# CDCgov/NowcastAutoGP

Hardware: AMD Instinct MI355X
Metric: particle-logml/s (fit+forecast hot path: covariance assembly + Cholesky + logml + predictive per (particle, scenario) item), n=2048 64-particle SMC (higher is better)
Workload: dtype f64

## Files before the change

### nowcastautogp_amd/csrc/ngp_col_kernels.h

```cpp
#pragma once
#include <algorithm>

#include "ngp_mfma.h"

namespace ngp {

struct NoProbe {
    __device__ __forceinline__ void mark(int) {}
    template <class T>
    __device__ __forceinline__ void mark_after(int, T) {}
    __device__ __forceinline__ void drain() {}
    __device__ __forceinline__ void emit_diag(int, int, int) {}
    __device__ __forceinline__ void emit_col(int, int, int, int, int, int, bool) {}
    __device__ __forceinline__ void begin(int, int, int) {}
    __device__ __forceinline__ void sweep(int) {}
};

__device__ __forceinline__ void sqrt_and_rcp(double a, double &d, double &r) {
    double y = __builtin_amdgcn_rsq(a);
    const double h = 0.5 * a;
    y = y * fma(-h * y, y, 1.5);
    y = y * fma(-h * y, y, 1.5);
    d = a * y;
    d = fma(fma(-d, d, a), 0.5 * y, d);
    r = fma(fma(-d, y, 1.0), y, y);
}

__device__ __forceinline__ int tri(int r, int c) { return ((r * (r + 1)) >> 1) + c; }
constexpr int TRI = NB * (NB + 1) / 2;

template <class Probe = NoProbe>
__global__ __launch_bounds__(256, 4) void chol_diag_kernel(JobGeom g, ChunkPtrs p, int j, int k0) {
    __shared__ double Mt[TRI];
    __shared__ double Lt[TRI];
    __shared__ double pan[NB][4];
    __shared__ double dblk[16];
    __shared__ double dinvd[4];
    __shared__ double rdg[NB];
    __shared__ double logs[NB];
    __shared__ double Ts[TB][TB + 1];
    __shared__ int bad;
    const int item = blockIdx.x;
    const int tid = threadIdx.x, lane = tid & 63;
    const int wave = __builtin_amdgcn_readfirstlane(tid >> 6);
    const long ld = g.ld;
    double *Lit = p.L + (long)item * g.item_stride;
    double *Lj = Lit + (long)j * NB * ld;
    const int kmax = j * NB;
    const int r16 = lane & 15, q = lane >> 4;
    const int wr = wave >> 1, wc = wave & 1;
    Probe probe;
    probe.mark_after(0, lane);

    if (tid == 0) bad = 0;

    if (!(wr == 0 && wc == 1)) {
        double acc4[2][2][4];
#pragma unroll
        for (int a = 0; a < 2; ++a)
#pragma unroll
            for (int b = 0; b < 2; ++b)
#pragma unroll
                for (int r = 0; r < 4; ++r) acc4[a][b][r] = 0.0;
        const double *pa = Lj + (long)(32 * wr + r16) * ld + 2 * q;
        const double *pb = Lj + (long)(32 * wc + r16) * ld + 2 * q;
        double kt[2][2][4];
#pragma unroll
        for (int mt = 0; mt < 2; ++mt)
#pragma unroll
            for (int nt = 0; nt < 2; ++nt)
#pragma unroll
                for (int s = 0; s < 4; ++s)
                    kt[mt][nt][s] = Lj[(long)(32 * wr + 16 * mt + q + 4 * s) * ld + kmax +
                                       32 * wc + 16 * nt + r16];
        for (int kc = k0; kc < kmax; kc += 16) {
            double a[2][4], b[2][4];
#pragma unroll
            for (int u = 0; u < 2; ++u) {
                const f64x2 alo = *reinterpret_cast<const f64x2 *>(pa + (long)u * 16 * ld + kc);
                const f64x2 ahi = *reinterpret_cast<const f64x2 *>(pa + (long)u * 16 * ld + kc + 8);
                const f64x2 blo = *reinterpret_cast<const f64x2 *>(pb + (long)u * 16 * ld + kc);
                const f64x2 bhi = *reinterpret_cast<const f64x2 *>(pb + (long)u * 16 * ld + kc + 8);
                a[u][0] = alo.x; a[u][1] = alo.y; a[u][2] = ahi.x; a[u][3] = ahi.y;
                b[u][0] = blo.x; b[u][1] = blo.y; b[u][2] = bhi.x; b[u][3] = bhi.y;
            }
#pragma unroll
            for (int s = 0; s < 4; ++s)
#pragma unroll
                for (int nt = 0; nt < 2; ++nt) {
                    const Rot4 br = rot4(b[nt][s]);
#pragma unroll
                    for (int mt = 0; mt < 2; ++mt) mfma16_as_4(acc4[mt][nt], a[mt][s], br);
                }
        }
        f64x4 acc[2][2];
#pragma unroll
        for (int a = 0; a < 2; ++a)
#pragma unroll
            for (int b = 0; b < 2; ++b) acc[a][b] = to_d16(acc4[a][b]);
#pragma unroll
        for (int mt = 0; mt < 2; ++mt)
#pragma unroll
            for (int nt = 0; nt < 2; ++nt)
#pragma unroll
                for (int s = 0; s < 4; ++s) {
                    const int M = 32 * wr + 16 * mt + q + 4 * s, N = 32 * wc + 16 * nt + r16;
                    if (M >= N) Mt[tri(M, N)] = kt[mt][nt][s] - acc[mt][nt][s];
                }
    }
    __syncthreads();
    probe.mark_after(1, lane);

    const int bi = tid >> 4, bj = tid & 15;
    {
        double a[4][4];
#pragma unroll
        for (int r = 0; r < 4; ++r)
#pragma unroll
            for (int c = 0; c < 4; ++c) {
                const int R = 4 * bi + r, C = 4 * bj + c;
                a[r][c] = (R >= C) ? Mt[tri(R, C)] : 0.0;
            }
        for (int kb = 0; kb < NB / 4; ++kb) {
            if (bi == kb && bj == kb) {
                double dks[4];
#pragma unroll
                for (int kc = 0; kc < 4; ++kc) {
                    const double akk = a[kc][kc];
                    double dk, inv;
                    sqrt_and_rcp(akk, dk, inv);
                    if (!(akk > 0.0) && bad == 0) bad = 4 * kb + kc + 1;
                    dks[kc] = dk;
                    dinvd[kc] = inv;
                    rdg[4 * kb + kc] = inv;
#pragma unroll
                    for (int r = 0; r < 4; ++r)
                        if (r > kc) a[r][kc] *= inv;
#pragma unroll
                    for (int c = 0; c < 4; ++c)
                        if (c > kc) {
#pragma unroll
                            for (int r = 0; r < 4; ++r)
                                if (r >= c) a[r][c] -= a[r][kc] * a[c][kc];
                        }
                }
#pragma unroll
                for (int r = 0; r < 4; ++r)
#pragma unroll
                    for (int c = 0; c < 4; ++c) {
                        if (r == c) a[r][c] = dks[r];
                        if (c > r) a[r][c] = 0.0;
                        dblk[4 * r + c] = a[r][c];
                    }
            }
            __syncthreads();
            if (bj == kb && bi > kb) {
#pragma unroll
                for (int c = 0; c < 4; ++c) {
                    const double inv = dinvd[c];
#pragma unroll
                    for (int r = 0; r < 4; ++r) {
                        double v = a[r][c];
#pragma unroll
                        for (int pp = 0; pp < 4; ++pp)
                            if (pp < c) v -= a[r][pp] * dblk[4 * c + pp];
                        a[r][c] = v * inv;
                    }
                }
#pragma unroll
                for (int r = 0; r < 4; ++r)
#pragma unroll
                    for (int c = 0; c < 4; ++c) pan[4 * bi + r][c] = a[r][c];
            }
            __syncthreads();
            if (bj > kb && bi >= bj) {
                double li[4][4], lj[4][4];
#pragma unroll
                for (int r = 0; r < 4; ++r)
#pragma unroll
                    for (int pp = 0; pp < 4; ++pp) {
                        li[r][pp] = pan[4 * bi + r][pp];
                        lj[r][pp] = pan[4 * bj + r][pp];
                    }
#pragma unroll
                for (int pp = 0; pp < 4; ++pp)
#pragma unroll
                    for (int r = 0; r < 4; ++r)
#pragma unroll
                        for (int c = 0; c < 4; ++c) a[r][c] -= li[r][pp] * lj[c][pp];
            }
        }
#pragma unroll
        for (int r = 0; r < 4; ++r) {
            const int R = 4 * bi + r;
            f64x2 lo, hi;
            lo.x = (R >= 4 * bj) ? a[r][0] : 0.0;
            lo.y = (R >= 4 * bj + 1) ? a[r][1] : 0.0;
            hi.x = (R >= 4 * bj + 2) ? a[r][2] : 0.0;
            hi.y = (R >= 4 * bj + 3) ? a[r][3] : 0.0;
            double *dst = Lj + (long)R * ld + kmax + 4 * bj;
            *reinterpret_cast<f64x2 *>(dst) = lo;
            *reinterpret_cast<f64x2 *>(dst + 2) = hi;
#pragma unroll
            for (int c = 0; c < 4; ++c)
                if (R >= 4 * bj + c) Lt[tri(R, 4 * bj + c)] = a[r][c];
        }
    }
    __syncthreads();
    probe.mark_after(2, lane);
    if (tid < NB) logs[tid] = log(Lt[tri(tid, tid)]);

    if (tid < NB) {
        const int b = tid >> 4, c = tid & 15;
        double x[TB];
#pragma unroll
        for (int i = 0; i < TB; ++i) {
            double sum = (i == c) ? 1.0 : 0.0;
            int off = tri(TB * b + i, TB * b);
            if (i > 0) asm volatile("" : "+v"(off) : "v"(x[i - 1]));
            const double *lrow = &Lt[off];
#pragma unroll
            for (int pp = 0; pp < i; ++pp) sum -= lrow[pp] * x[pp];
            x[i] = sum * rdg[TB * b + i];
        }
#pragma unroll
        for (int i = 0; i < TB; ++i)
            if (i >= c) Mt[tri(TB * b + i, TB * b + c)] = x[i];
    }
    __syncthreads();
    probe.mark_after(3, lane);
    {
        const int ra = tid >> 4, cb = tid & 15;
        for (int dist = 1; dist < NB / TB; ++dist)
            for (int ct = dist; ct < NB / TB; ++ct) {
                const int jt = ct - dist;
                double t = 0.0;
                for (int kt = jt; kt < ct; ++kt)
#pragma unroll
                    for (int pp = 0; pp < TB; ++pp) {
                        const double mv = Mt[tri(TB * kt + pp, TB * jt + cb)];
                        t += Lt[tri(TB * ct + ra, TB * kt + pp)] * ((kt > jt || pp >= cb) ? mv : 0.0);
                    }
                Ts[ra][cb] = t;
                __syncthreads();
                double mv = 0.0;
#pragma unroll
                for (int pp = 0; pp < TB; ++pp) {
                    const double md = Mt[tri(TB * ct + ra, TB * ct + pp)];
                    mv -= ((pp <= ra) ? md : 0.0) * Ts[pp][cb];
                }
                Mt[tri(TB * ct + ra, TB * jt + cb)] = mv;
                __syncthreads();
            }
    }
    probe.mark_after(4, lane);
    {
        double *dv = p.dinv + (long)item * (NB * NB);
        for (int e = tid; e < NB * NB; e += 256) {
            const int strip = e >> 6, l = e & 63;
            const int cb4 = strip >> 2, jt = strip & 3;
            const int R = 4 * cb4 + (l & 3), C = 16 * jt + 4 * ((l >> 2) & 3) + (l >> 4);
            dv[e] = (R >= C) ? Mt[tri(R, C)] : 0.0;
        }
    }
    if (tid == 0) {
        double s = 0.0;
        for (int k = 0; k < NB; ++k) s += logs[k];
        p.logdet[item] += s;
        if (bad && p.info[item] == 0) p.info[item] = kmax + bad;
    }
    probe.mark_after(5, lane);
    probe.emit_diag(j, tid, item);
}

template <int NF>
struct Frag8 {
    f64x2 v[NF];
};
template <int NF>
__device__ __forceinline__ void load_frag8(Frag8<NF> &f, const double *p, long ld) {
#pragma unroll
    for (int u = 0; u < NF; ++u) f.v[u] = *reinterpret_cast<const f64x2 *>(p + (long)u * 16 * ld);
}
template <int NA>
__device__ __forceinline__ void mfma_frag8(double (&acc)[NA][4][4], const Frag8<NA> &a,
                                           const Frag8<4> &b) {
#pragma unroll
    for (int it = 0; it < 4; ++it) {
        const Rot4 br = rot4(b.v[it].x);
#pragma unroll
        for (int jt = 0; jt < NA; ++jt) mfma16_as_4(acc[jt][it], a.v[jt].x, br);
    }
#pragma unroll
    for (int it = 0; it < 4; ++it) {
        const Rot4 br = rot4(b.v[it].y);
#pragma unroll
        for (int jt = 0; jt < NA; ++jt) mfma16_as_4(acc[jt][it], a.v[jt].y, br);
    }
}

template <int NA>
__device__ __forceinline__ void gemm_rows(double (&acc)[NA][4][4], const double *pa,
                                          const double *pb, long ld, int k0, int k1) {
    if (k1 <= k0) return;
    Frag8<NA> a0, a1;
    Frag8<4> b0, b1;
    load_frag8(a0, pa + k0, ld);
    load_frag8(b0, pb + k0, ld);
    for (int kc = k0; kc < k1; kc += 16) {
        load_frag8(a1, pa + kc + 8, ld);
        load_frag8(b1, pb + kc + 8, ld);
        mfma_frag8(acc, a0, b0);
        if (kc + 16 < k1) {
            load_frag8(a0, pa + kc + 16, ld);
            load_frag8(b0, pb + kc + 16, ld);
        }
        mfma_frag8(acc, a1, b1);
    }
}

constexpr int EPI_PITCH = 66;
constexpr int EPI_M_BYTES = NB * NB * 8;
constexpr int EPI_WAVE_BYTES = 16 * EPI_PITCH * 8;
constexpr int EPI_LDS_BYTES = EPI_M_BYTES + 4 * EPI_WAVE_BYTES;

__device__ __forceinline__ void stage_mstrips(double *lds_m, const double *mstrips, int tid) {
#pragma unroll
    for (int i = 0; i < 8; ++i) {
        const int idx = tid + 256 * i;
        reinterpret_cast<f64x2 *>(lds_m)[idx] = reinterpret_cast<const f64x2 *>(mstrips)[idx];
    }
}

template <bool SHADOW = false, bool SYNTH = false, class Probe = NoProbe, bool KROWS = false>
__device__ __forceinline__ void solve_and_store_lds(const double (*acc4)[4][4], double *Lr,
                                                    const double *lds_m, long ld, int kmax,
                                                    int lane, double *buf, Probe &probe,
                                                    float *Lr32 = nullptr,
                                                    float *tmax_out = nullptr, int synth = 0,
                                                    const double *ksl = nullptr, int nit = 4) {
    double amax = 0.0;
    const int n16 = lane & 15, isub = lane >> 4;
    const int jj0 = 4 * (n16 >> 2) + isub;
    const double *ksl0 = ksl ? ksl + 15 - jj0 : nullptr;
    f64x2 kvr[8];
    double kvp[4][4];
    const int hrow = lane >> 5, c2 = 2 * (lane & 31);
    bool from_rows = KROWS && ksl0 == nullptr;
    if constexpr (SYNTH) from_rows = from_rows && synth == 0;
    auto k_elems = [&](int it, double (&kv)[4][4]) {
        if (ksl0) {
#pragma unroll
            for (int jt = 0; jt < 4; ++jt)
#pragma unroll
                for (int r = 0; r < 4; ++r)
                    kv[jt][r] = ksl0[((n16 + 4 * r) & 15) + 16 * (it - jt + 3)];
            return;
        }
        if constexpr (SYNTH) {
            if (synth) {
#pragma unroll
                for (int jt = 0; jt < 4; ++jt)
#pragma unroll
                    for (int r = 0; r < 4; ++r) {
                        const int i = 16 * it + ((n16 + 4 * r) & 15);
                        kv[jt][r] = (synth == 2 && i == 16 * jt + jj0) ? 1.0 : 0.0;
                    }
                return;
            }
        }
        if constexpr (!KROWS) {
#pragma unroll
            for (int jt = 0; jt < 4; ++jt)
#pragma unroll
                for (int r = 0; r < 4; ++r) {
                    const int i = 16 * it + ((n16 + 4 * r) & 15);
                    kv[jt][r] = Lr[(long)i * ld + kmax + 16 * jt + jj0];
                }
        }
    };
    auto load_k = [&](int it) {
        if constexpr (KROWS) {
            if (!from_rows) return;
#pragma unroll
            for (int i = 0; i < 8; ++i)
                kvr[i] = *reinterpret_cast<const f64x2 *>(Lr + (long)(16 * it + 2 * i + hrow) * ld + kmax + c2);
        } else {
            k_elems(it, kvp);
        }
    };
    auto take_k = [&](int it, double (&kv)[4][4]) {
        if constexpr (KROWS) {
            if (!from_rows) {
                k_elems(it, kv);
                return;
            }
#pragma unroll
            for (int i = 0; i < 8; ++i)
                *reinterpret_cast<f64x2 *>(buf + (2 * i + hrow) * EPI_PITCH + c2) = kvr[i];
#pragma unroll
            for (int jt = 0; jt < 4; ++jt)
#pragma unroll
                for (int r = 0; r < 4; ++r)
                    kv[jt][r] = buf[((n16 + 4 * r) & 15) * EPI_PITCH + 16 * jt + jj0];
        } else {
#pragma unroll
            for (int jt = 0; jt < 4; ++jt)
#pragma unroll
                for (int r = 0; r < 4; ++r) kv[jt][r] = kvp[jt][r];
        }
    };
    load_k(0);
#pragma unroll
    for (int it = 0; it < 4; ++it) {
        if (it >= nit) break;
        double c4[4][4];
        take_k(it, c4);
#pragma unroll
        for (int jt = 0; jt < 4; ++jt)
#pragma unroll
            for (int r = 0; r < 4; ++r) c4[jt][r] = c4[jt][r] - acc4[jt][it][r];
        probe.mark_after(12 + 3 * it, c4[3][3] + c4[0][0] + c4[1][2] + c4[2][1]);
        if (it + 1 < nit) load_k(it + 1);
        double ms[2][4];
        ms[0][0] = lds_m[lane];
#pragma unroll
        for (int cb4 = 0; cb4 < 16; ++cb4) {
            const int ct = cb4 >> 2;
            if (cb4 + 1 < 16) {
#pragma unroll
                for (int jt = 0; jt <= ((cb4 + 1) >> 2); ++jt)
                    ms[(cb4 + 1) & 1][jt] = lds_m[((cb4 + 1) * 4 + jt) * 64 + lane];
            }
            double R[4] = {0.0, 0.0, 0.0, 0.0};
#pragma unroll
            for (int jt = 0; jt <= ct; ++jt) {
#pragma unroll
                for (int r = 0; r < 4; ++r) R[r] = mfma4(ms[cb4 & 1][jt], c4[jt][r], R[r]);
            }
            double x = R[0];
            x += dpp_f64<ROW_ROR4, 0xF>(R[1], R[1]);
            x += dpp_f64<ROW_ROR8, 0xF>(R[2], R[2]);
            x += dpp_f64<ROW_ROR12, 0xF>(R[3], R[3]);
            buf[n16 * EPI_PITCH + 4 * cb4 + isub] = x;
        }
        probe.mark_after(13 + 3 * it, it);
#pragma unroll
        for (int w = 0; w < 8; ++w) {
            const int idx = w * 64 + lane, row = idx >> 5, cp = idx & 31;
            const f64x2 v = *reinterpret_cast<const f64x2 *>(buf + row * EPI_PITCH + 2 * cp);
            *reinterpret_cast<f64x2 *>(Lr + (long)(16 * it + row) * ld + kmax + 2 * cp) = v;
            if constexpr (SHADOW) {
                typedef float f32x2 __attribute__((ext_vector_type(2)));
                f32x2 vf;
                vf.x = (float)v.x;
                vf.y = (float)v.y;
                *reinterpret_cast<f32x2 *>(Lr32 + (long)(16 * it + row) * ld + kmax + 2 * cp) = vf;
                amax = fmax(amax, fmax(fabs(v.x), fabs(v.y)));
            }
        }
        probe.mark_after(14 + 3 * it, it);
        __builtin_amdgcn_sched_barrier(0);
    }
    if constexpr (SHADOW) {
#pragma unroll
        for (int off = 32; off > 0; off >>= 1) amax = fmax(amax, __shfl_xor(amax, off, 64));
        if (lane == 0) *tmax_out = __double2float_ru(amax);
    }
}

__device__ __forceinline__ void subtract_in_place_perm(double *rows, long ld, int c0,
                                                       const double (*acc4)[4][4], int lane,
                                                       bool fresh = false,
                                                       const double *ksl = nullptr, int nit = 4) {
    const int n16 = lane & 15, isub = lane >> 4;
    const int jj0 = 4 * (n16 >> 2) + isub;
    double *base = rows + c0 + jj0;
    long roff[4];
#pragma unroll
    for (int r = 0; r < 4; ++r) roff[r] = (long)((n16 + 4 * r) & 15) * ld;
    if (ksl) {
        const double *ksl0 = ksl + 15 - jj0;
#pragma unroll
        for (int it = 0; it < 4; ++it)
#pragma unroll
            for (int jt = 0; jt < 4; ++jt)
#pragma unroll
                for (int r = 0; r < 4; ++r)
                    base[(long)(16 * it) * ld + roff[r] + 16 * jt] =
                        ksl0[((n16 + 4 * r) & 15) + 16 * (it - jt + 3)] - acc4[jt][it][r];
        return;
    }
    if (fresh) {
#pragma unroll
        for (int it = 0; it < 4; ++it)
#pragma unroll
            for (int jt = 0; jt < 4; ++jt)
#pragma unroll
                for (int r = 0; r < 4; ++r)
                    base[(long)(16 * it) * ld + roff[r] + 16 * jt] = -acc4[jt][it][r];
        return;
    }
    double v[2][4][4];
#pragma unroll
    for (int jt = 0; jt < 4; ++jt)
#pragma unroll
        for (int r = 0; r < 4; ++r) v[0][jt][r] = base[roff[r] + 16 * jt];
#pragma unroll
    for (int it = 0; it < 4; ++it) {
        if (it >= nit) break;
        if (it + 1 < nit) {
#pragma unroll
            for (int jt = 0; jt < 4; ++jt)
#pragma unroll
                for (int r = 0; r < 4; ++r)
                    v[(it + 1) & 1][jt][r] = base[(long)(16 * (it + 1)) * ld + roff[r] + 16 * jt];
        }
#pragma unroll
        for (int jt = 0; jt < 4; ++jt)
#pragma unroll
            for (int r = 0; r < 4; ++r)
                base[(long)(16 * it) * ld + roff[r] + 16 * jt] = v[it & 1][jt][r] - acc4[jt][it][r];
    }
}

__device__ __forceinline__ void subtract_in_place_rows(double *rows, long ld, int c0,
                                                       const double (*acc4)[4][4], int lane,
                                                       double *tl, bool fresh = false,
                                                       const double *ksl = nullptr, int nit = 4) {
    const int n16 = lane & 15, isub = lane >> 4;
    const int jj0 = 4 * (n16 >> 2) + isub;
    const int hrow = lane >> 5, c2 = 2 * (lane & 31);
    double *base = rows + c0 + c2;
    auto load_rows = [&](int it, f64x2 (&kv)[8]) {
        if (ksl) {
#pragma unroll
            for (int i = 0; i < 8; ++i) {
                const int d = 63 + 16 * it + 2 * i + hrow - c2;
                kv[i].x = ksl[d];
                kv[i].y = ksl[d - 1];
            }
        } else if (fresh) {
#pragma unroll
            for (int i = 0; i < 8; ++i) kv[i].x = kv[i].y = 0.0;
        } else {
#pragma unroll
            for (int i = 0; i < 8; ++i)
                kv[i] = *reinterpret_cast<const f64x2 *>(base + (long)(16 * it + 2 * i + hrow) * ld);
        }
    };
    f64x2 kv[2][8];
    load_rows(0, kv[0]);
#pragma unroll
    for (int it = 0; it < 4; ++it) {
        if (it >= nit) break;
        if (it + 1 < nit) load_rows(it + 1, kv[(it + 1) & 1]);
#pragma unroll
        for (int jt = 0; jt < 4; ++jt)
#pragma unroll
            for (int r = 0; r < 4; ++r)
                tl[((n16 + 4 * r) & 15) * EPI_PITCH + 16 * jt + jj0] = acc4[jt][it][r];
#pragma unroll
        for (int i = 0; i < 8; ++i) {
            const f64x2 a = *reinterpret_cast<const f64x2 *>(tl + (2 * i + hrow) * EPI_PITCH + c2);
            f64x2 o;
            o.x = kv[it & 1][i].x - a.x;
            o.y = kv[it & 1][i].y - a.y;
            *reinterpret_cast<f64x2 *>(base + (long)(16 * it + 2 * i + hrow) * ld) = o;
        }
    }
}

__device__ __forceinline__ void struct_slice(double *ksl, const JobGeom &g, const ChunkPtrs &p,
                                             int item, int row0, int col0, int lane) {
    const double *tab = p.tab + (long)item * g.maxstat * g.R;
    const int d0 = row0 - col0 - 63;
    ksl[lane] = tab[(long)g.toep * (d0 + lane)];
    if (lane < 63) ksl[64 + lane] = tab[(long)g.toep * (d0 + 64 + lane)];
}
constexpr int TOEP_LDS_BYTES = 4 * 128 * 8;

struct ColStep {
    int j;
    int k0;
    int nmain;
    int ntiles;
    int groups;
    int splits;
    int first_touch;
    double c32, jitter;
};
__device__ __forceinline__ long tmax_index(const JobGeom &g, int row_tile, int col) {
    return (long)row_tile * g.nb0 + col;
}

template <bool MIXED, bool IDENT = false, bool TOEP = false>
__global__ __launch_bounds__(256, 2) void chol_col_kernel(JobGeom g, ChunkPtrs p, int Bc,
                                                          ColStep st) {
    __shared__ __attribute__((aligned(16))) char epi[EPI_LDS_BYTES + (TOEP ? TOEP_LDS_BYTES : 0)];
    const int wg = blockIdx.x;
    const int xcd = wg & 7, idx = wg >> 3;
    const int slot = (idx / st.groups) * 8 + xcd;
    const int grp = idx % st.groups;
    if (slot >= Bc) return;
    const int item = p.items ? p.items[slot] : slot;
    const int tid = threadIdx.x, lane = tid & 63;
    const int wave = __builtin_amdgcn_readfirstlane(tid >> 6);
    const int tile = grp * 4 + wave;
    bool valid = tile < st.ntiles;
    int kbeg = st.k0;
    int synth = 0;
    if constexpr (IDENT) {
        if (valid && tile >= st.nmain) {
            const int a = tile - st.nmain;
            if (a < g.nb0) {
                if (a > st.j) valid = false;
                else if (a * NB > kbeg) kbeg = a * NB;
                synth = (a == st.j) ? 2 : 1;
            }
        }
    }

    const int j = st.j;
    const long ld = g.ld;
    double *Lit = p.L + (long)item * g.item_stride;
    const int kmax = j * NB;
    const int r16 = lane & 15, q = lane >> 4;

    double acc4[4][4][4];
#pragma unroll
    for (int a = 0; a < 4; ++a)
#pragma unroll
        for (int b = 0; b < 4; ++b)
#pragma unroll
            for (int r = 0; r < 4; ++r) acc4[a][b][r] = 0.0;

    const int vt = valid ? tile : 0;
    const long rowbase = (vt < st.nmain) ? (long)(j + 1 + vt) * NB
                                         : (long)g.n0 + (long)(vt - st.nmain) * NB;
    double *Lr = Lit + rowbase * ld;
    const double *Lj = Lit + (long)j * NB * ld;
    const double *pa = Lj + (long)r16 * ld + 2 * q;
    const double *pb = Lr + (long)r16 * ld + 2 * q;
    if (valid) gemm_rows<4>(acc4, pa, pb, ld, kbeg, kmax);
    const double *ksl = nullptr;
    if constexpr (TOEP) {
        if (valid && tile < st.nmain && prog_structure(p.progs + item)) {
            double *sl = reinterpret_cast<double *>(epi + EPI_LDS_BYTES) + wave * 128;
            struct_slice(sl, g, p, item, (int)rowbase, kmax, lane);
            ksl = sl;
        }
    }
    stage_mstrips(reinterpret_cast<double *>(epi), p.dinv + (long)item * (NB * NB), tid);
    __syncthreads();
    if (!valid) return;
    NoProbe probe;
    if constexpr (MIXED) {
        const int rt = (tile < st.nmain) ? j + 1 + tile : g.nb0 + (tile - st.nmain);
        solve_and_store_lds<true>(
            acc4, Lr, reinterpret_cast<const double *>(epi), ld, kmax, lane,
            reinterpret_cast<double *>(epi + EPI_M_BYTES + wave * EPI_WAVE_BYTES), probe,
            p.L32 + (long)item * g.item_stride + rowbase * ld,
            p.tmax + (long)item * (g.nb0 + g.naux_pad / NB) * g.nb0 + tmax_index(g, rt, j));
    } else {
        solve_and_store_lds<false, IDENT>(
            acc4, Lr, reinterpret_cast<const double *>(epi), ld, kmax, lane,
            reinterpret_cast<double *>(epi + EPI_M_BYTES + wave * EPI_WAVE_BYTES), probe, nullptr,
            nullptr, synth, ksl);
    }
}

template <bool MIXED, class Probe = NoProbe, bool IDENT = false>
__global__ __launch_bounds__(256, 2) void chol_col_thin_kernel(JobGeom g, ChunkPtrs p, int Bc,
                                                               ColStep st) {
    constexpr int A_BYTES = NB * NB * 8;
    constexpr int TAIL = (4 * EPI_WAVE_BYTES > A_BYTES) ? 4 * EPI_WAVE_BYTES : A_BYTES;
    __shared__ __attribute__((aligned(1024))) char smem[EPI_M_BYTES + TAIL];
    typedef __attribute__((address_space(3))) void *lds_ptr;
    const int wg = blockIdx.x;
    const int xcd = wg & 7, idx = wg >> 3;
    const int slot = (idx / st.groups) * 8 + xcd;
    const int grp = idx % st.groups;
    if (slot >= Bc) return;
    const int item = p.items ? p.items[slot] : slot;
    const int tid = threadIdx.x, lane = tid & 63;
    const int wave = __builtin_amdgcn_readfirstlane(tid >> 6);
    const int tile = grp * 4 + wave;
    bool valid = tile < st.ntiles;
    const int j = st.j;
    const int kmax = j * NB, k0 = kmax - NB;
    bool update = true;
    int synth = 0;
    if constexpr (IDENT) {
        if (valid && tile >= st.nmain) {
            const int a = tile - st.nmain;
            if (a < g.nb0) {
                if (a > j) valid = false;
                else if (a * NB > k0) update = false;
                if (a == j) synth = 2;
            }
        }
    }
    const long ld = g.ld;
    double *Lit = p.L + (long)item * g.item_stride;
    const int r16 = lane & 15, q = lane >> 4;
    Probe probe;
    probe.mark_after(0, lane);

    {
        const __amdgpu_buffer_rsrc_t rl = __builtin_amdgcn_make_buffer_rsrc(
            Lit, 0, (int)(g.item_stride * (long)sizeof(double)), 0x00020000);
        const __amdgpu_buffer_rsrc_t rm = __builtin_amdgcn_make_buffer_rsrc(
            p.dinv + (long)item * (NB * NB), 0, NB * NB * 8, 0x00020000);
        const int rbit = lane >> 5, sl = lane & 31;
#pragma unroll
        for (int i = 0; i < 8; ++i) {
            const int key = (2 * i + rbit) & 7;
            const unsigned voff = (unsigned)((rbit * ld + 2 * (sl ^ key)) * 8);
            const unsigned soff = (unsigned)__builtin_amdgcn_readfirstlane(
                (int)((((long)kmax + 2 * (8 * wave + i)) * ld + k0) * 8));
            lds_ptr dst = (lds_ptr)(smem + EPI_M_BYTES + (8 * wave + i) * 1024);
            __builtin_amdgcn_raw_ptr_buffer_load_lds(rl, dst, 16, voff, soff, 0, 0);
        }
#pragma unroll
        for (int i = 0; i < 8; ++i) {
            lds_ptr dst = (lds_ptr)(smem + (8 * wave + i) * 1024);
            __builtin_amdgcn_raw_ptr_buffer_load_lds(rm, dst, 16, (unsigned)(lane * 16),
                                                     (unsigned)((8 * wave + i) * 1024), 0, 0);
        }
    }

    double acc4[4][4][4];
#pragma unroll
    for (int a = 0; a < 4; ++a)
#pragma unroll
        for (int b = 0; b < 4; ++b)
#pragma unroll
            for (int r = 0; r < 4; ++r) acc4[a][b][r] = 0.0;

    const int vt = valid ? tile : 0;
    const long rowbase = (vt < st.nmain) ? (long)(j + 1 + vt) * NB
                                         : (long)g.n0 + (long)(vt - st.nmain) * NB;
    double *Lr = Lit + rowbase * ld;
    const double *pb = Lr + (long)r16 * ld + k0 + 2 * q;
    const bool mult = valid && update;
    Frag8<4> b[4];
    if (mult) {
#pragma unroll
        for (int sg = 0; sg < 4; ++sg) load_frag8(b[sg], pb + 8 * sg, ld);
    }
    __syncthreads();
    probe.mark_after(1, lane);
    if (mult) {
        const char *Ab = smem + EPI_M_BYTES + r16 * 512;
        const int key = r16 & 7;
#pragma unroll
        for (int sg = 0; sg < 8; ++sg) {
            Frag8<4> a;
#pragma unroll
            for (int u = 0; u < 4; ++u)
                a.v[u] = *reinterpret_cast<const f64x2 *>(Ab + u * (16 * 512) +
                                                          (((4 * sg + q) ^ key) << 4));
            mfma_frag8(acc4, a, b[sg & 3]);
            if (sg + 4 < 8) load_frag8(b[sg & 3], pb + 8 * (sg + 4), ld);
        }
    }
    probe.mark_after(2, acc4[0][0][0] + acc4[3][3][3]);
    __syncthreads();
    probe.mark_after(3, lane);
    probe.mark_after(4, lane);
    if (!valid) return;
    double *buf = reinterpret_cast<double *>(smem + EPI_M_BYTES + wave * EPI_WAVE_BYTES);
    if constexpr (MIXED) {
        const int rt = (tile < st.nmain) ? j + 1 + tile : g.nb0 + (tile - st.nmain);
        solve_and_store_lds<true, false, Probe, true>(
            acc4, Lr, reinterpret_cast<const double *>(smem), ld, kmax, lane, buf, probe,
            p.L32 + (long)item * g.item_stride + rowbase * ld,
            p.tmax + (long)item * (g.nb0 + g.naux_pad / NB) * g.nb0 + tmax_index(g, rt, j));
    } else {
        int nit = (tile >= st.nmain && g.naux - NB * (tile - st.nmain) <= 16) ? 1 : 4;
        if (IDENT && tile < st.nmain && g.n_real - NB * (j + 1 + tile) <= 16) nit = 1;
        solve_and_store_lds<false, IDENT, Probe, true>(acc4, Lr, reinterpret_cast<const double *>(smem), ld,
                                          kmax, lane, buf, probe, nullptr, nullptr, synth, nullptr,
                                          nit);
    }
    probe.mark_after(5, lane);
    probe.drain();
    probe.mark_after(6, lane);
    probe.emit_col(j, lane, wg, wave, item, tile, true);
}

constexpr int LDS_KC = 16;

typedef float f32x4 __attribute__((ext_vector_type(4)));
typedef float f32x16 __attribute__((ext_vector_type(16)));


template <bool MIXED, class Probe = NoProbe, bool IDENT = false, int SPLITK = 0>
__global__ __launch_bounds__(256, 2) void chol_col_glds_kernel(JobGeom g, ChunkPtrs p, int Bc,
                                                               ColStep st) {
    constexpr int ROWB = 128, BLKB = 8 * ROWB + 128, STAGE = 32 * BLKB;
    auto row_off = [](int row) { return (row >> 3) * BLKB + (row & 7) * ROWB; };
    __shared__ __attribute__((aligned(1024))) char smem[2 * STAGE];
    typedef __attribute__((address_space(3))) void *lds_ptr;

    const int wg = blockIdx.x;
    const int xcd = wg & 7, idx = wg >> 3;
    const int per_item = SPLITK == 1 ? st.groups * st.splits : st.groups;
    const int slot = (idx / per_item) * 8 + xcd;
    const int grp = SPLITK == 1 ? (idx % per_item) / st.splits : idx % st.groups;
    const int piece = SPLITK == 1 ? (idx % per_item) % st.splits : 0;
    if (slot >= Bc) return;
    const int item = (MIXED && p.order) ? p.order[slot] : slot;
    const int tid = threadIdx.x, lane = tid & 63;
    const int wave = __builtin_amdgcn_readfirstlane(tid >> 6);
    const int ltile = wave >> 1, col = wave & 1;
    const int tile0 = grp * 2;
    const int tile = tile0 + ltile;
    bool valid = tile < st.ntiles;

    const int j = st.j;
    Probe probe;
    probe.mark(0);
    const long ld = g.ld;
    double *Lit = p.L + (long)item * g.item_stride;
    const int kmax = j * NB;
    bool structured = false;
    if constexpr (!MIXED && !IDENT) {
        if (g.toep && st.first_touch && valid && tile < st.nmain && !(col && tile == 0))
            structured = prog_structure(p.progs + item) != 0;
    }
    int kbeg = st.k0;
    int synth = 0;
    if constexpr (IDENT) {
        const int a = tile - st.nmain;
        if (tile < st.ntiles && a >= 0 && a < g.nb0) synth = (a == j) ? 2 : 1;
    }
    if (IDENT && tile0 >= st.nmain) {
        int kfirst = kmax + 1;
#pragma unroll
        for (int u = 0; u < 2; ++u) {
            const int a = tile0 + u - st.nmain;
            if (tile0 + u >= st.ntiles) continue;
            const int ks = (a >= g.nb0) ? st.k0 : (a > j) ? kmax + 1 : max(st.k0, a * NB);
            kfirst = min(kfirst, ks);
        }
        if (kfirst > kmax) return;
        kbeg = kfirst;
        const int a = tile - st.nmain;
        if (valid && a < g.nb0 && a > j) valid = false;
    }
    int nit = 4;
    if constexpr (!MIXED && SPLITK == 0) {
        if (IDENT && !valid) nit = 0;
        else if (valid && tile >= st.nmain && g.naux - NB * (tile - st.nmain) <= 16) nit = 1;
        else if (IDENT && valid && tile < st.nmain && g.n_real - NB * (j + 1 + tile) <= 16) nit = 1;
    }
    const int r16 = lane & 15, q = lane >> 4;
    auto tile_row0 = [&](int t) -> long {
        if (t >= st.ntiles) t = st.ntiles - 1;
        return (t < st.nmain) ? (long)(j + 1 + t) * NB : (long)g.n0 + (long)(t - st.nmain) * NB;
    };
    const __amdgpu_buffer_rsrc_t rsrc = __builtin_amdgcn_make_buffer_rsrc(
        Lit, 0, (int)(g.item_stride * (long)sizeof(double)), 0x00020000);
    long src_row0;
    if (wave < 2) src_row0 = (long)j * NB + 64 * wave;
    else src_row0 = tile_row0(tile0 + (wave - 2));
    const unsigned soff_base = (unsigned)__builtin_amdgcn_readfirstlane((int)(src_row0 * ld * 8));
    const unsigned row_step8 = (unsigned)(8 * ld * 8);
    const unsigned voff_even = (unsigned)(((lane >> 3) * ld + 2 * ((lane & 7) ^ ((lane >> 4) & 7))) * 8);
    const unsigned voff_odd = (unsigned)(((lane >> 3) * ld + 2 * ((lane & 7) ^ ((4 + (lane >> 4)) & 7))) * 8);
    auto stage = [&](int buf, int k) {
        const unsigned kb = (unsigned)k * 8u;
#pragma unroll
        for (int i = 0; i < 8; ++i) {
            lds_ptr dst = (lds_ptr)(smem + buf * STAGE + (8 * wave + i) * BLKB);
            __builtin_amdgcn_raw_ptr_buffer_load_lds(rsrc, dst, 16, (i & 1) ? voff_odd : voff_even,
                                                     soff_base + i * row_step8 + kb, 0, 0);
        }
    };
    unsigned a_addr[4], b_addr[4][4];
    {
        const int arow = 64 * col + r16;
        const int akey = (r16 >> 1) & 7;
#pragma unroll
        for (int s = 0; s < 4; ++s)
            a_addr[s] = (unsigned)(row_off(arow) + (((2 * s + (q >> 1)) ^ akey) << 4) + (q & 1) * 8);
#pragma unroll
        for (int r = 0; r < 4; ++r) {
            const int rr = (r16 + 4 * r) & 15;
            const int brow = 128 + 64 * ltile + rr;
            const int bkey = (rr >> 1) & 7;
#pragma unroll
            for (int s = 0; s < 4; ++s)
                b_addr[r][s] =
                    (unsigned)(row_off(brow) + (((2 * s + (q >> 1)) ^ bkey) << 4) + (q & 1) * 8);
        }
    }

    double acc4[4][4][4];
#pragma unroll
    for (int a = 0; a < 4; ++a)
#pragma unroll
        for (int b = 0; b < 4; ++b)
#pragma unroll
            for (int r = 0; r < 4; ++r) acc4[a][b][r] = 0.0;

    auto mult64 = [&](const char *buf, auto nit_c) {
        constexpr int NIT = decltype(nit_c)::value;
#pragma unroll
        for (int s = 0; s < 4; ++s) {
            double a[4];
#pragma unroll
            for (int u = 0; u < 4; ++u)
                a[u] = *reinterpret_cast<const double *>(buf + a_addr[s] + u * 2 * BLKB);
#pragma unroll
            for (int it = 0; it < NIT; ++it) {
                Rot4 br;
                br.r0 = *reinterpret_cast<const double *>(buf + b_addr[0][s] + it * 2 * BLKB);
                br.r1 = *reinterpret_cast<const double *>(buf + b_addr[1][s] + it * 2 * BLKB);
                br.r2 = *reinterpret_cast<const double *>(buf + b_addr[2][s] + it * 2 * BLKB);
                br.r3 = *reinterpret_cast<const double *>(buf + b_addr[3][s] + it * 2 * BLKB);
#pragma unroll
                for (int jt = 0; jt < 4; ++jt) mfma16_as_4(acc4[jt][it], a[jt], br);
            }
        }
    };

    if constexpr (SPLITK == 2) {
    } else if constexpr (!MIXED) {
        int nchunks = (kmax - kbeg) / LDS_KC;
        if constexpr (SPLITK == 1) {
            const int per = (nchunks + st.splits - 1) / st.splits;
            const int c0 = min(piece * per, nchunks);
            nchunks = min(c0 + per, nchunks) - c0;
            kbeg += c0 * LDS_KC;
        }
        if (nchunks > 0) {
            stage(0, kbeg);
            __syncthreads();
            if (IDENT && nit == 0) {
                for (int c = 0; c < nchunks; ++c) {
                    if (c + 1 < nchunks) stage((c & 1) ^ 1, kbeg + (c + 1) * LDS_KC);
                    __syncthreads();
                }
            } else if (nit == 1) {
                for (int c = 0; c < nchunks; ++c) {
                    const int cur = c & 1;
                    if (c + 1 < nchunks) stage(cur ^ 1, kbeg + (c + 1) * LDS_KC);
                    mult64(smem + cur * STAGE, std::integral_constant<int, 1>{});
                    __syncthreads();
                }
            } else {
                for (int c = 0; c < nchunks; ++c) {
                    const int cur = c & 1;
                    if (c + 1 < nchunks) stage(cur ^ 1, kbeg + (c + 1) * LDS_KC);
                    mult_chunk_pipelined<2 * BLKB>(acc4, smem + cur * STAGE, a_addr, b_addr);
                    __syncthreads();
                    if (c == 0) probe.mark(1);
                    if (c == nchunks / 2) probe.mark(2);
                }
            }
        }
    } else {
        const int nkt = j;
        const int nbt = g.nb0 + g.naux_pad / NB;
        const float *tm = p.tmax + (long)item * nbt * g.nb0;
        const int t1 = min(tile0 + 1, st.ntiles - 1);
        const int rt0 = (tile0 < st.nmain) ? j + 1 + tile0 : g.nb0 + (tile0 - st.nmain);
        const int rt1 = (t1 < st.nmain) ? j + 1 + t1 : g.nb0 + (t1 - st.nmain);
        const double lim = st.c32 * (p.progs[item].noise + st.jitter);
        unsigned long long m32lo, m32hi;
        {
            bool c[2];
#pragma unroll
            for (int h = 0; h < 2; ++h) {
                const int kt = lane + 64 * h;
                c[h] = false;
                if (kt < nkt) {
                    const float ta = fmaxf(tm[tmax_index(g, j, kt)], tm[tmax_index(g, j + 1, kt)]);
                    const float tb = fmaxf(tm[tmax_index(g, rt0, kt)], tm[tmax_index(g, rt1, kt)]);
                    c[h] = (double)ta * (double)tb <= lim;
                }
            }
            m32lo = __ballot(c[0]);
            m32hi = __ballot(c[1]);
        }
        const unsigned long long inlo = nkt >= 64 ? ~0ull : ((1ull << nkt) - 1ull);
        const unsigned long long inhi = nkt <= 64 ? 0ull : (nkt >= 128 ? ~0ull : ((1ull << (nkt - 64)) - 1ull));
        unsigned long long m64lo = inlo & ~m32lo, m64hi = inhi & ~m32hi;
        const int n32 = __popcll(m32lo) + __popcll(m32hi);
        const int n64 = __popcll(m64lo) + __popcll(m64hi);
        if (tid == 0 && p.mixcnt) {
            const unsigned nv = (unsigned)(2 * min(2, st.ntiles - tile0));
            atomicAdd(p.mixcnt + 2 * item, nv * (unsigned)n32);
            atomicAdd(p.mixcnt + 2 * item + 1, nv * (unsigned)n64);
        }
        auto pop = [](unsigned long long &lo, unsigned long long &hi) -> int {
            if (lo) {
                const int b = __builtin_ctzll(lo);
                lo &= lo - 1;
                return b;
            }
            const int b = __builtin_ctzll(hi);
            hi &= hi - 1;
            return 64 + b;
        };

        if (n32 > 0) {
            const __amdgpu_buffer_rsrc_t rsrc32 = __builtin_amdgcn_make_buffer_rsrc(
                p.L32 + (long)item * g.item_stride, 0, (int)(g.item_stride * (long)sizeof(float)),
                0x00020000);
            const unsigned soff32 = (unsigned)__builtin_amdgcn_readfirstlane((int)(src_row0 * ld * 4));
            const unsigned row_step32 = (unsigned)(8 * ld * 4);
            const unsigned v32_even = (unsigned)((lane >> 3) * ld * 4 + 16 * ((lane & 7) ^ ((lane >> 4) & 7)));
            const unsigned v32_odd = (unsigned)((lane >> 3) * ld * 4 + 16 * ((lane & 7) ^ ((4 + (lane >> 4)) & 7)));
            auto stage32 = [&](int buf, int k) {
                const unsigned kb = (unsigned)k * 4u;
#pragma unroll
                for (int i = 0; i < 8; ++i) {
                    lds_ptr dst = (lds_ptr)(smem + buf * STAGE + (8 * wave + i) * BLKB);
                    __builtin_amdgcn_raw_ptr_buffer_load_lds(rsrc32, dst, 16,
                                                             (i & 1) ? v32_odd : v32_even,
                                                             soff32 + i * row_step32 + kb, 0, 0);
                }
            };
            const int r32 = lane & 31, h = lane >> 5;
            unsigned a32[2][4], b32[2][4];
#pragma unroll
            for (int blk = 0; blk < 2; ++blk) {
                const int arow = 64 * col + 32 * blk + r32;
                const int brow = 128 + 64 * ltile + 32 * blk + r32;
#pragma unroll
                for (int u = 0; u < 4; ++u) {
                    a32[blk][u] = (unsigned)(row_off(arow) + (((2 * u + h) ^ ((arow >> 1) & 7)) << 4));
                    b32[blk][u] = (unsigned)(row_off(brow) + (((2 * u + h) ^ ((brow >> 1) & 7)) << 4));
                }
            }
            f32x16 acc32[2][2];
            double acc64p[2][2][16];
#pragma unroll
            for (int a = 0; a < 2; ++a)
#pragma unroll
                for (int b = 0; b < 2; ++b)
#pragma unroll
                    for (int v = 0; v < 16; ++v) {
                        acc32[a][b][v] = 0.f;
                        acc64p[a][b][v] = 0.0;
                    }
            unsigned long long lo = m32lo, hi = m32hi;
            const int nch = 2 * n32;
            int kt_cur = pop(lo, hi), sub = 1;
            stage32(0, kt_cur * NB);
            __syncthreads();
            for (int c = 0; c < nch; ++c) {
                const int cur = c & 1;
                if (c + 1 < nch) {
                    if (sub == 2) {
                        kt_cur = pop(lo, hi);
                        sub = 0;
                    }
                    stage32(cur ^ 1, kt_cur * NB + 32 * sub);
                    ++sub;
                }
                const char *buf = smem + cur * STAGE;
#pragma unroll
                for (int u = 0; u < 4; ++u) {
                    f32x4 av[2], bv[2];
#pragma unroll
                    for (int blk = 0; blk < 2; ++blk) {
                        av[blk] = *reinterpret_cast<const f32x4 *>(buf + a32[blk][u]);
                        bv[blk] = *reinterpret_cast<const f32x4 *>(buf + b32[blk][u]);
                    }
#pragma unroll
                    for (int e = 0; e < 4; ++e)
#pragma unroll
                        for (int a = 0; a < 2; ++a)
#pragma unroll
                            for (int b = 0; b < 2; ++b)
                                acc32[a][b] = __builtin_amdgcn_mfma_f32_32x32x2f32(
                                    av[a][e], bv[b][e], acc32[a][b], 0, 0, 0);
                }
                if (c & 1) {
#pragma unroll
                    for (int a = 0; a < 2; ++a)
#pragma unroll
                        for (int b = 0; b < 2; ++b)
#pragma unroll
                            for (int v = 0; v < 16; ++v) {
                                acc64p[a][b][v] += (double)acc32[a][b][v];
                                acc32[a][b][v] = 0.f;
                            }
                }
                __syncthreads();
            }
            constexpr int P64 = 65;
            double *t64 = reinterpret_cast<double *>(smem) + wave * (32 * P64);
            static_assert(4 * 32 * P64 * 8 <= 2 * STAGE, "hand-over tiles must fit the stage buffers");
            const int jj0 = 4 * (r16 >> 2) + q;
#pragma unroll
            for (int a = 0; a < 2; ++a) {
#pragma unroll
                for (int b = 0; b < 2; ++b)
#pragma unroll
                    for (int v = 0; v < 16; ++v)
                        t64[((v & 3) + 8 * (v >> 2) + 4 * h) * P64 + 32 * b + r32] = acc64p[a][b][v];
                __syncthreads();
#pragma unroll
                for (int jl = 0; jl < 2; ++jl)
#pragma unroll
                    for (int it = 0; it < 4; ++it)
#pragma unroll
                        for (int r = 0; r < 4; ++r)
                            acc4[2 * a + jl][it][r] =
                                t64[(16 * jl + jj0) * P64 + 16 * it + ((r16 + 4 * r) & 15)];
                __syncthreads();
            }
        }
        if (n64 > 0) {
            unsigned long long lo = m64lo, hi = m64hi;
            const int nch = 4 * n64;
            int kt_cur = pop(lo, hi), sub = 1;
            stage(0, kt_cur * NB);
            __syncthreads();
            for (int c = 0; c < nch; ++c) {
                const int cur = c & 1;
                if (c + 1 < nch) {
                    if (sub == 4) {
                        kt_cur = pop(lo, hi);
                        sub = 0;
                    }
                    stage(cur ^ 1, kt_cur * NB + LDS_KC * sub);
                    ++sub;
                }
                mult_chunk_pipelined<2 * BLKB>(acc4, smem + cur * STAGE, a_addr, b_addr);
                __syncthreads();
            }
        }
    }
    if constexpr (SPLITK == 1) {
        double *mine = p.splitk_part +
                       ((((long)slot * SPLITK_SLOTS + (long)grp * st.splits + piece) * 4 + wave) *
                        (64 * 64)) + lane;
#pragma unroll
        for (int jt = 0; jt < 4; ++jt)
#pragma unroll
            for (int it = 0; it < 4; ++it)
#pragma unroll
                for (int r = 0; r < 4; ++r) mine[((jt * 4 + it) * 4 + r) * 64] = acc4[jt][it][r];
        return;
    }
    if constexpr (SPLITK == 2) {
        const double *part = p.splitk_part +
                             ((((long)slot * SPLITK_SLOTS + (long)grp * st.splits) * 4 + wave) *
                              (64 * 64)) + lane;
#pragma unroll
        for (int jt = 0; jt < 4; ++jt)
#pragma unroll
            for (int it = 0; it < 4; ++it)
#pragma unroll
                for (int r = 0; r < 4; ++r) acc4[jt][it][r] = part[((jt * 4 + it) * 4 + r) * 64];
        for (int q2 = 1; q2 < st.splits; ++q2) {
            const double *pq = part + (long)q2 * 4 * (64 * 64);
            double v[4][4][4];
#pragma unroll
            for (int jt = 0; jt < 4; ++jt)
#pragma unroll
                for (int it = 0; it < 4; ++it)
#pragma unroll
                    for (int r = 0; r < 4; ++r) v[jt][it][r] = pq[((jt * 4 + it) * 4 + r) * 64];
#pragma unroll
            for (int jt = 0; jt < 4; ++jt)
#pragma unroll
                for (int it = 0; it < 4; ++it)
#pragma unroll
                    for (int r = 0; r < 4; ++r) acc4[jt][it][r] += v[jt][it][r];
        }
    }
    static_assert(EPI_LDS_BYTES + TOEP_LDS_BYTES <= 2 * STAGE,
                  "epilogue LDS must fit the stage buffers");
    probe.mark(3);
    const double *ksl = nullptr;
    if (structured) {
        double *sl = reinterpret_cast<double *>(smem + EPI_LDS_BYTES) + wave * 128;
        struct_slice(sl, g, p, item, (int)tile_row0(tile), col ? kmax + NB : kmax, lane);
        ksl = sl;
    }
    stage_mstrips(reinterpret_cast<double *>(smem), p.dinv + (long)item * (NB * NB), tid);
    __syncthreads();
    probe.mark(4);
    if (!valid) return;

    double *Lr = Lit + tile_row0(tile) * ld;
    if (col) {
        subtract_in_place_rows(Lr, ld, (j + 1) * NB, acc4, lane,
                               reinterpret_cast<double *>(smem + EPI_M_BYTES + wave * EPI_WAVE_BYTES),
                               IDENT && synth != 0, ksl, nit);
    } else if constexpr (MIXED) {
        const int rt = (tile < st.nmain) ? j + 1 + tile : g.nb0 + (tile - st.nmain);
        solve_and_store_lds<true>(
            acc4, Lr, reinterpret_cast<const double *>(smem), ld, kmax, lane,
            reinterpret_cast<double *>(smem + EPI_M_BYTES + wave * EPI_WAVE_BYTES), probe,
            p.L32 + (long)item * g.item_stride + tile_row0(tile) * ld,
            p.tmax + (long)item * (g.nb0 + g.naux_pad / NB) * g.nb0 + tmax_index(g, rt, j));
    } else {
        solve_and_store_lds<false, IDENT>(
            acc4, Lr, reinterpret_cast<const double *>(smem), ld, kmax, lane,
            reinterpret_cast<double *>(smem + EPI_M_BYTES + wave * EPI_WAVE_BYTES), probe, nullptr,
            nullptr, synth, ksl, nit);
    }
    probe.mark(5);
    probe.drain();
    probe.mark(6);
    probe.emit_col(j, lane, wg, wave, item, tile, false);
}

template <class Probe>
void launch_chol_diag_t(const JobGeom &g, const ChunkPtrs &p, int Bc, int j, int k0, hipStream_t s) {
    hipLaunchKernelGGL(chol_diag_kernel<Probe>, dim3(Bc), dim3(256), 0, s, g, p, j, k0);
}

template <class Probe>
void launch_chol_col_t(const JobGeom &g, const ChunkPtrs &p, int Bc, int j, int mode, int k0,
                     hipStream_t s, const DevSpec *sp) {
    ColStep st{};
    const bool mixed = p.L32 != nullptr && sp != nullptr;
    if (mixed) {
        st.c32 = sp->mixed_tau / (64.0 * 5.9604644775390625e-08);
        st.jitter = sp->jitter;
    }
    st.j = j;
    st.k0 = k0;
    st.nmain = (mode == COL_AUX) ? 0 : g.nb0 - 1 - j;
    st.ntiles = st.nmain + g.naux_pad / NB;
    if (st.ntiles <= 0) return;
    const int bpad = (Bc + 7) / 8 * 8;
    const dim3 blk(256);
    st.first_touch = (mode == COL_FAT || (mode == COL_FULL && k0 == 0 && j == 0)) ? 1 : 0;
    if (mode == COL_FAT) {
        st.groups = (st.ntiles + 1) / 2;
        const dim3 grid(st.groups * bpad);
        int splits = 1;
        if (!mixed && !g.aux_identity && p.splitk_part) splits = splitk_count(st.groups, j * NB / LDS_KC, Bc);
        st.splits = std::max(splits, 1);
        if (splits >= 2) {
            hipLaunchKernelGGL((chol_col_glds_kernel<false, Probe, false, 1>),
                               dim3(st.groups * splits * bpad), blk, 0, s, g, p, Bc, st);
            hipLaunchKernelGGL((chol_col_glds_kernel<false, Probe, false, 2>), grid, blk, 0, s, g, p,
                               Bc, st);
        } else if (mixed)
            hipLaunchKernelGGL((chol_col_glds_kernel<true, Probe>), grid, blk, 0, s, g, p, Bc, st);
        else if (g.aux_identity)
            hipLaunchKernelGGL((chol_col_glds_kernel<false, Probe, true>), grid, blk, 0, s, g, p, Bc, st);
        else
            hipLaunchKernelGGL((chol_col_glds_kernel<false, Probe>), grid, blk, 0, s, g, p, Bc, st);
    } else if (mode == COL_THIN && k0 == j * NB - NB && j > 0) {
        st.groups = (st.ntiles + 3) / 4;
        const dim3 grid(st.groups * bpad);
        if (mixed)
            hipLaunchKernelGGL((chol_col_thin_kernel<true, Probe>), grid, blk, 0, s, g, p, Bc, st);
        else if (g.aux_identity)
            hipLaunchKernelGGL((chol_col_thin_kernel<false, Probe, true>), grid, blk, 0, s, g, p, Bc, st);
        else
            hipLaunchKernelGGL((chol_col_thin_kernel<false, Probe>), grid, blk, 0, s, g, p, Bc, st);
    } else {
        st.groups = (st.ntiles + 3) / 4;
        const dim3 grid(st.groups * bpad);
        if (mixed)
            hipLaunchKernelGGL(chol_col_kernel<true>, grid, blk, 0, s, g, p, Bc, st);
        else if (g.aux_identity)
            hipLaunchKernelGGL((chol_col_kernel<false, true>), grid, blk, 0, s, g, p, Bc, st);
        else if (g.toep && st.first_touch)
            hipLaunchKernelGGL((chol_col_kernel<false, false, true>), grid, blk, 0, s, g, p, Bc, st);
        else
            hipLaunchKernelGGL(chol_col_kernel<false>, grid, blk, 0, s, g, p, Bc, st);
    }
}

}
```

Measured before the change: 15800.

## Hand the last triangular-solve pass to the sibling column wave

The solve wave (col 0) now finishes only three of the four 16-row passes of the panel triangular solve. It writes the accumulator for the last pass into the LDS tile of its sibling column wave, which runs that pass before its own trailing-update subtraction. The aim is to balance the epilogue between the two waves of a tile. It also skips the trailing subtraction when there is nothing to accumulate, and in mixed mode it merges the shadow amax across the two waves through LDS with an extra block barrier. The cost is an extra __syncthreads and LDS traffic, and it reuses the sibling's LDS tile as the hand-over buffer.

Result: faster. 16020 (median of 6 runs) (+1.4%).

```diff
diff --git a/nowcastautogp_amd/csrc/ngp_col_kernels.h b/nowcastautogp_amd/csrc/ngp_col_kernels.h
--- a/nowcastautogp_amd/csrc/ngp_col_kernels.h
+++ b/nowcastautogp_amd/csrc/ngp_col_kernels.h
@@ -332,13 +332,18 @@
     }
 }
 
-template <bool SHADOW = false, bool SYNTH = false, class Probe = NoProbe, bool KROWS = false>
-__device__ __forceinline__ void solve_and_store_lds(const double (*acc4)[4][4], double *Lr,
-                                                    const double *lds_m, long ld, int kmax,
-                                                    int lane, double *buf, Probe &probe,
-                                                    float *Lr32 = nullptr,
-                                                    float *tmax_out = nullptr, int synth = 0,
-                                                    const double *ksl = nullptr, int nit = 4) {
+constexpr int EPI_HAND_PASS = 3;
+template <bool SHADOW = false, bool SYNTH = false, class Probe = NoProbe, bool KROWS = false,
+          bool HAND = false>
+__device__ __forceinline__ double solve_and_store_lds(const double (*acc4)[4][4], double *Lr,
+                                                      const double *lds_m, long ld, int kmax,
+                                                      int lane, double *buf, Probe &probe,
+                                                      float *Lr32 = nullptr,
+                                                      float *tmax_out = nullptr, int synth = 0,
+                                                      const double *ksl = nullptr, int nit = 4,
+                                                      const double *hand = nullptr) {
+    static_assert(!(HAND && KROWS), "the row form of K' goes through the tile the hand-over is in");
+    constexpr int IT0 = HAND ? EPI_HAND_PASS : 0;
     double amax = 0.0;
     const int n16 = lane & 15, isub = lane >> 4;
     const int jj0 = 4 * (n16 >> 2) + isub;
@@ -410,16 +415,19 @@
                 for (int r = 0; r < 4; ++r) kv[jt][r] = kvp[jt][r];
         }
     };
-    load_k(0);
-#pragma unroll
-    for (int it = 0; it < 4; ++it) {
+    load_k(IT0);
+#pragma unroll
+    for (int it = IT0; it < 4; ++it) {
         if (it >= nit) break;
         double c4[4][4];
         take_k(it, c4);
 #pragma unroll
         for (int jt = 0; jt < 4; ++jt)
 #pragma unroll
-            for (int r = 0; r < 4; ++r) c4[jt][r] = c4[jt][r] - acc4[jt][it][r];
+            for (int r = 0; r < 4; ++r) {
+                if constexpr (HAND) c4[jt][r] = c4[jt][r] - hand[(4 * jt + r) * 64 + lane];
+                else c4[jt][r] = c4[jt][r] - acc4[jt][it][r];
+            }
         probe.mark_after(12 + 3 * it, c4[3][3] + c4[0][0] + c4[1][2] + c4[2][1]);
         if (it + 1 < nit) load_k(it + 1);
         double ms[2][4];
@@ -465,8 +473,9 @@
     if constexpr (SHADOW) {
 #pragma unroll
         for (int off = 32; off > 0; off >>= 1) amax = fmax(amax, __shfl_xor(amax, off, 64));
-        if (lane == 0) *tmax_out = __double2float_ru(amax);
-    }
+        if (tmax_out && lane == 0) *tmax_out = __double2float_ru(amax);
+    }
+    return amax;
 }
 
 __device__ __forceinline__ void subtract_in_place_perm(double *rows, long ld, int c0,
@@ -825,10 +834,12 @@
     const long ld = g.ld;
     double *Lit = p.L + (long)item * g.item_stride;
     const int kmax = j * NB;
-    bool structured = false;
+    bool structured = false, sib_structured = false;
     if constexpr (!MIXED && !IDENT) {
-        if (g.toep && st.first_touch && valid && tile < st.nmain && !(col && tile == 0))
-            structured = prog_structure(p.progs + item) != 0;
+        if (g.toep && st.first_touch && valid && tile < st.nmain) {
+            sib_structured = prog_structure(p.progs + item) != 0;
+            structured = sib_structured && !(col && tile == 0);
+        }
     }
     int kbeg = st.k0;
     int synth = 0;
@@ -1177,37 +1188,67 @@
                     for (int r = 0; r < 4; ++r) acc4[jt][it][r] += v[jt][it][r];
         }
     }
-    static_assert(EPI_LDS_BYTES + TOEP_LDS_BYTES <= 2 * STAGE,
+    static_assert(EPI_LDS_BYTES + TOEP_LDS_BYTES + 2 * 8 <= 2 * STAGE,
                   "epilogue LDS must fit the stage buffers");
+    static_assert(16 * 64 * 8 <= EPI_WAVE_BYTES, "S' of one pass must fit a wave's LDS tile");
     probe.mark(3);
-    const double *ksl = nullptr;
+    double *wtile = reinterpret_cast<double *>(smem + EPI_M_BYTES + wave * EPI_WAVE_BYTES);
+    const bool hand_over = valid && nit == 4;
+    const double *ksl = nullptr, *sib_ksl = nullptr;
     if (structured) {
         double *sl = reinterpret_cast<double *>(smem + EPI_LDS_BYTES) + wave * 128;
         struct_slice(sl, g, p, item, (int)tile_row0(tile), col ? kmax + NB : kmax, lane);
         ksl = sl;
     }
+    if (col && sib_structured) sib_ksl = reinterpret_cast<double *>(smem + EPI_LDS_BYTES) + (wave - 1) * 128;
+    if (!col && hand_over) {
+        double *hand = reinterpret_cast<double *>(smem + EPI_M_BYTES + (wave + 1) * EPI_WAVE_BYTES);
+#pragma unroll
+        for (int jt = 0; jt < 4; ++jt)
+#pragma unroll
+            for (int r = 0; r < 4; ++r) hand[(4 * jt + r) * 64 + lane] = acc4[jt][EPI_HAND_PASS][r];
+    }
     stage_mstrips(reinterpret_cast<double *>(smem), p.dinv + (long)item * (NB * NB), tid);
     __syncthreads();
     probe.mark(4);
-    if (!valid) return;
+    if constexpr (!MIXED) {
+        if (!valid) return;
+    }
 
     double *Lr = Lit + tile_row0(tile) * ld;
-    if (col) {
-        subtract_in_place_rows(Lr, ld, (j + 1) * NB, acc4, lane,
-                               reinterpret_cast<double *>(smem + EPI_M_BYTES + wave * EPI_WAVE_BYTES),
-                               IDENT && synth != 0, ksl, nit);
-    } else if constexpr (MIXED) {
-        const int rt = (tile < st.nmain) ? j + 1 + tile : g.nb0 + (tile - st.nmain);
-        solve_and_store_lds<true>(
-            acc4, Lr, reinterpret_cast<const double *>(smem), ld, kmax, lane,
-            reinterpret_cast<double *>(smem + EPI_M_BYTES + wave * EPI_WAVE_BYTES), probe,
-            p.L32 + (long)item * g.item_stride + tile_row0(tile) * ld,
-            p.tmax + (long)item * (g.nb0 + g.naux_pad / NB) * g.nb0 + tmax_index(g, rt, j));
+    const double *lds_m = reinterpret_cast<const double *>(smem);
+    const int nown = hand_over ? EPI_HAND_PASS : nit;
+    const bool no_sum = SPLITK == 0 && (MIXED ? j == 0 : kmax <= kbeg);
+    if constexpr (MIXED) {
+        double *xch = reinterpret_cast<double *>(smem + EPI_LDS_BYTES + TOEP_LDS_BYTES);
+        float *Lr32 = p.L32 + (long)item * g.item_stride + tile_row0(tile) * ld;
+        double amax = 0.0;
+        if (valid && col) {
+            if (hand_over)
+                amax = solve_and_store_lds<true, false, Probe, false, true>(
+                    acc4, Lr, lds_m, ld, kmax, lane, wtile, probe, Lr32, nullptr, 0, nullptr, 4, wtile);
+            if (lane == 0) xch[ltile] = amax;
+            if (!no_sum) subtract_in_place_rows(Lr, ld, (j + 1) * NB, acc4, lane, wtile, false, nullptr, nit);
+        } else if (valid) {
+            amax = solve_and_store_lds<true, false, Probe>(acc4, Lr, lds_m, ld, kmax, lane, wtile,
+                                                           probe, Lr32, nullptr, 0, nullptr, nown);
+        }
+        __syncthreads();
+        if (valid && !col && lane == 0) {
+            const int rt = (tile < st.nmain) ? j + 1 + tile : g.nb0 + (tile - st.nmain);
+            p.tmax[(long)item * (g.nb0 + g.naux_pad / NB) * g.nb0 + tmax_index(g, rt, j)] =
+                __double2float_ru(fmax(amax, xch[ltile]));
+        }
+    } else if (col) {
+        if (hand_over)
+            solve_and_store_lds<false, IDENT, Probe, false, true>(
+                acc4, Lr, lds_m, ld, kmax, lane, wtile, probe, nullptr, nullptr, synth, sib_ksl, 4, wtile);
+        const bool fresh = IDENT && synth != 0;
+        if (!(no_sum && !fresh && ksl == nullptr))
+            subtract_in_place_rows(Lr, ld, (j + 1) * NB, acc4, lane, wtile, fresh, ksl, nit);
     } else {
-        solve_and_store_lds<false, IDENT>(
-            acc4, Lr, reinterpret_cast<const double *>(smem), ld, kmax, lane,
-            reinterpret_cast<double *>(smem + EPI_M_BYTES + wave * EPI_WAVE_BYTES), probe, nullptr,
-            nullptr, synth, ksl, nit);
+        solve_and_store_lds<false, IDENT, Probe>(acc4, Lr, lds_m, ld, kmax, lane, wtile, probe, nullptr,
+                                                 nullptr, synth, ksl, nown);
     }
     probe.mark(5);
     probe.drain();
```
